# qiskit-community/adapt-aqc

Measured on AMD Instinct MI355X. Metric: overlap+gradient evals/sec, 50-qubit MPS chi=64, 1/2/4/8 MI355X, higher is better.
Workload: dtype c128

## Files before the change

### adaptaqc_amd/_lib.py

```python
import atexit
import ctypes
import os
import threading

import numpy as np

_HERE = os.path.dirname(os.path.abspath(__file__))
LIB_PATH = os.environ.get("AQC_LIB") or os.path.join(_HERE, "libaqchip.so")

OP_DTYPE = np.dtype(
    [("nq", "<i4"), ("q0", "<i4"), ("q1", "<i4"), ("flags", "<i4"), ("m", "<f8", (32,))], align=True
)
assert OP_DTYPE.itemsize == 272
OP_KRAUS1 = 1
OP_MEASURE1 = 2
OP_KRAUS2 = 3

EXPORTS = (
    "aqc_last_error", "aqc_version", "aqc_init", "aqc_finalize", "aqc_timing_enable",
    "aqc_timing_query", "aqc_timing_reset",
    "aqc_sv_create", "aqc_sv_destroy", "aqc_sv_reset", "aqc_sv_copy", "aqc_sv_apply", "aqc_sv_plan",
    "aqc_sv_amp0", "aqc_sv_z_all", "aqc_sv_get", "aqc_sv_set",
    "aqc_mps_create", "aqc_mps_destroy", "aqc_mps_set_truncation", "aqc_mps_set_vidal",
    "aqc_mps_get_vidal", "aqc_mps_get_dims", "aqc_mps_copy", "aqc_mps_copy_batch", "aqc_mps_apply",
    "aqc_mps_apply_batch", "aqc_mps_apply_sort_batch", "aqc_mps_apply_sort_batch_async", "aqc_mps_apply_batch_async", "aqc_mps_check_batch", "aqc_mps_sort", "aqc_mps_sort_batch", "aqc_mps_overlap_zero",
    "aqc_mps_overlap_zero_batch", "aqc_mps_dot", "aqc_mps_z_all", "aqc_mps_amps_hw1", "aqc_mps_z_all_batch", "aqc_mps_z_sum_batch", "aqc_mps_zero_hw1_batch",
    "aqc_mps_amps_hw1_batch",
    "aqc_pair_grads", "aqc_pair_grads_batch", "aqc_argmax_scaled", "aqc_argmax_scaled_batch", "aqc_mps_jacobi_stats",
    "aqc_mps_set_jacobi_tol", "aqc_mps_set_jacobi_stop", "aqc_mps_set_fused_chain", "aqc_mps_chain_ticks", "aqc_svd_debug",
    "aqc_sv_pair_rdms", "aqc_mps_pair_rdms", "aqc_mps_pair_rdms_batch", "aqc_entanglement_measures",
    "aqc_sv_transition", "aqc_mps_product_fit", "aqc_mps_set_svd_path", "aqc_svd_gram_ticks", "aqc_bj_ticks",
    "aqc_sweep_set_chain_mode", "aqc_stream_join", "aqc_stream_wait", "aqc_svd_gram_stats", "aqc_env_ticks",
    "aqc_comm_unique_id", "aqc_comm_init", "aqc_comm_destroy", "aqc_comm_rank", "aqc_allgather_f64",
    "aqc_allgather_f64_host", "aqc_allreduce_max_f64", "aqc_svd_gram_big_stats", "aqc_svd_gram_big_ticks",
    "aqc_gb_set_spin_limit", "aqc_gb_set_tail", "aqc_gb_set_stages", "aqc_debug_hog", "aqc_pool_stats",
    "aqc_scratch_stats", "aqc_mps_set_chain_epilogue", "aqc_mps_chain_epilogue_stats",
    "aqc_env_fallbacks", "aqc_env_set_single", "aqc_env_set_spin_limit",
    "aqc_sv_sample", "aqc_mps_sample", "aqc_sample_uniforms", "aqc_sv_traj_sample",
    "aqc_sv_traj_pair_tomo", "aqc_sv_traj_pauli_counts", "aqc_mps_traj_sample", "aqc_mps_traj_plan", "aqc_mps_traj_set_batch",
    "aqc_mps_traj_pair_tomo", "aqc_mps_traj_tomo_plan", "aqc_mps_traj_set_readout_batch",
    "aqc_sv_pauli_expect", "aqc_mps_pauli_expect", "aqc_mps_pauli_expect_batch",
    "aqc_pair_tomo_probs", "aqc_concurrence_bound_probs", "aqc_multinomial_counts", "aqc_tomo_fit",
)


class AqcError(RuntimeError):
    pass


_lock = threading.Lock()
_lib = None
_initialised_device = None

_P = ctypes.c_void_p
_I = ctypes.c_int
_D = ctypes.c_double
_DP = ctypes.POINTER(ctypes.c_double)
_IP = ctypes.POINTER(ctypes.c_int)

_SIGS = {
    "aqc_last_error": ([], ctypes.c_char_p),
    "aqc_version": ([], _I),
    "aqc_init": ([_I], _I),
    "aqc_finalize": ([], _I),
    "aqc_timing_enable": ([_I], _I),
    "aqc_timing_query": ([ctypes.c_char_p, _DP, ctypes.POINTER(ctypes.c_int64), _DP, _DP], _I),
    "aqc_timing_reset": ([], _I),
    "aqc_sv_create": ([_I, ctypes.POINTER(_P)], _I),
    "aqc_sv_destroy": ([_P], _I),
    "aqc_sv_reset": ([_P], _I),
    "aqc_sv_copy": ([_P, _P], _I),
    "aqc_sv_apply": ([_P, _P, _I], _I),
    "aqc_sv_plan": ([_I, _P, _I, _P], _I),
    "aqc_sv_amp0": ([_P, _DP, _DP], _I),
    "aqc_sv_z_all": ([_P, _DP], _I),
    "aqc_sv_get": ([_P, _P], _I),
    "aqc_sv_set": ([_P, _P], _I),
    "aqc_mps_create": ([_I, _I, _D, _I, ctypes.POINTER(_P)], _I),
    "aqc_mps_destroy": ([_P], _I),
    "aqc_mps_set_truncation": ([_P, _D, _I], _I),
    "aqc_mps_set_vidal": ([_P, _P, _P, _P], _I),
    "aqc_mps_get_vidal": ([_P, _P, _P, _P], _I),
    "aqc_mps_get_dims": ([_P, _P], _I),
    "aqc_mps_copy": ([_P, _P], _I),
    "aqc_mps_copy_batch": ([_P, _P, _I], _I),
    "aqc_mps_apply": ([_P, _P, _I], _I),
    "aqc_mps_apply_batch": ([_P, _I, _P, _P], _I),
    "aqc_mps_apply_sort_batch": ([_P, _I, _P, _P], _I),
    "aqc_mps_apply_sort_batch_async": ([_P, _I, _P, _P], _I),
    "aqc_mps_apply_batch_async": ([_P, _I, _P, _P], _I),
    "aqc_mps_check_batch": ([_P, _I], _I),
    "aqc_mps_sort": ([_P], _I),
    "aqc_mps_sort_batch": ([_P, _I], _I),
    "aqc_mps_overlap_zero": ([_P, _DP, _DP], _I),
    "aqc_mps_overlap_zero_batch": ([_P, _I, _P], _I),
    "aqc_mps_dot": ([_P, _P, _DP, _DP], _I),
    "aqc_mps_z_all": ([_P, _P], _I),
    "aqc_mps_amps_hw1": ([_P, _P], _I),
    "aqc_mps_z_all_batch": ([_P, _I, _P], _I),
    "aqc_mps_z_sum_batch": ([_P, _P, _I, _P], _I),
    "aqc_mps_zero_hw1_batch": ([_P, _P, _I, _P, _P], _I),
    "aqc_mps_amps_hw1_batch": ([_P, _I, _P], _I),
    "aqc_pair_grads": ([_P, _P, _P, _I, _P, _P, _P, _I, _P, _I], _I),
    "aqc_pair_grads_batch": ([_P, _I, _P, _P, _I, _P, _P, _P, _I, _P, _I], _I),
    "aqc_argmax_scaled": ([_P, _P, _I, _I, _IP], _I),
    "aqc_argmax_scaled_batch": ([_P, _I, _P, _I, _I, _P], _I),
    "aqc_mps_jacobi_stats": ([_P, _IP], _I),
    "aqc_mps_set_jacobi_tol": ([_D], _I),
    "aqc_mps_set_jacobi_stop": ([_D], _I),
    "aqc_mps_set_fused_chain": ([_I], _I),
    "aqc_mps_chain_ticks": ([_P], _I),
    "aqc_mps_set_chain_epilogue": ([_I], _I),
    "aqc_mps_chain_epilogue_stats": ([_P], _I),
    "aqc_svd_debug": ([_P, _I, _I, _I, _I, _P, _P, _P, _P], _I),
    "aqc_sv_pair_rdms": ([_P, _P, _I, _P], _I),
    "aqc_mps_pair_rdms": ([_P, _P, _I, _P], _I),
    "aqc_mps_pair_rdms_batch": ([_P, _I, _P, _I, _P, _I], _I),
    "aqc_entanglement_measures": ([_P, _I, _I, _P, _I], _I),
    "aqc_sv_transition": ([_P, _P, _I, _P], _I),
    "aqc_mps_product_fit": ([_P, _P, _I, _I, _I, _D, _DP, _IP], _I),
    "aqc_mps_set_svd_path": ([_I, _I], _I),
    "aqc_svd_gram_ticks": ([_P], _I),
    "aqc_bj_ticks": ([_P], _I),
    "aqc_sweep_set_chain_mode": ([_I], _I),
    "aqc_stream_join": ([_P], _I),
    "aqc_stream_wait": ([_P], _I),
    "aqc_svd_gram_stats": ([_P], _I),
    "aqc_env_ticks": ([_P], _I),
    "aqc_comm_unique_id": ([ctypes.c_char_p], _I),
    "aqc_comm_init": ([ctypes.c_char_p, _I, _I, ctypes.POINTER(_P)], _I),
    "aqc_comm_destroy": ([_P], _I),
    "aqc_comm_rank": ([_P, _IP, _IP], _I),
    "aqc_allgather_f64": ([_P, _P, _P, ctypes.c_size_t], _I),
    "aqc_allgather_f64_host": ([_P, _P, _P, ctypes.c_size_t], _I),
    "aqc_allreduce_max_f64": ([_P, _DP], _I),
    "aqc_svd_gram_big_stats": ([_P], _I),
    "aqc_svd_gram_big_ticks": ([_P], _I),
    "aqc_gb_set_spin_limit": ([_D], _I),
    "aqc_env_fallbacks": ([ctypes.POINTER(ctypes.c_longlong)], _I),
    "aqc_env_set_single": ([_I], _I),
    "aqc_env_set_spin_limit": ([_D], _I),
    "aqc_gb_set_tail": ([_I], _I),
    "aqc_gb_set_stages": ([_I], _I),
    "aqc_debug_hog": ([_I, _D], _I),
    "aqc_pool_stats": ([_P], _I),
    "aqc_scratch_stats": ([_P], _I),
    "aqc_sv_sample": ([_P, _I, ctypes.c_uint64, ctypes.c_uint64, _P, _P], _I),
    "aqc_mps_sample": ([_P, _I, ctypes.c_uint64, ctypes.c_uint64, _P, _P], _I),
    "aqc_sample_uniforms": ([ctypes.c_uint64, ctypes.c_uint64, _I, _I, _P], _I),
    "aqc_sv_traj_sample": ([_I, _P, _I, _I, ctypes.c_uint64, ctypes.c_uint64, _P, _P, _P], _I),
    "aqc_sv_traj_pair_tomo": ([_I, _P, _I, _P, _I, _P, _I, ctypes.c_uint64, ctypes.c_uint64, _P, _P, _P], _I),
    "aqc_sv_traj_pauli_counts": ([_I, _P, _I, _P, _I, _P, _I, ctypes.c_uint64, ctypes.c_uint64, _P, _P, _P, _P], _I),
    "aqc_mps_traj_sample": ([_I, _I, _D, _I, _P, _I, _I, ctypes.c_uint64, ctypes.c_uint64, _P, _P, _P], _I),
    "aqc_mps_traj_plan": ([_I, _P, _I, _P, _P, _I], _I),
    "aqc_mps_traj_set_batch": ([_I], _I),
    "aqc_mps_traj_pair_tomo": ([_I, _I, _D, _I, _P, _I, _P, _I, _P, _I, ctypes.c_uint64, ctypes.c_uint64, _P, _P, _P], _I),
    "aqc_mps_traj_tomo_plan": ([_I, _P, _I, _P, _P, _I], _I),
    "aqc_mps_traj_set_readout_batch": ([_I], _I),
    "aqc_sv_pauli_expect": ([_P, _P, _P, _I, _P], _I),
    "aqc_mps_pauli_expect": ([_P, _P, _I, _P], _I),
    "aqc_mps_pauli_expect_batch": ([_P, _I, _P, _I, _P], _I),
    "aqc_pair_tomo_probs": ([_P, _I, _P, _I], _I),
    "aqc_concurrence_bound_probs": ([_P, _I, _P, _I], _I),
    "aqc_multinomial_counts": ([_P, _I, _I, _I, ctypes.c_uint64, ctypes.c_uint64, _P, _P], _I),
    "aqc_tomo_fit": ([_P, _I, _P, _I], _I),
# ... 121 lines not shown
```

### adaptaqc_amd/csrc/mps.hip

```cpp
#include <algorithm>
#include <cmath>
#include <chrono>
#include <cstring>
#include <atomic>
#include <cstdlib>
#include <mutex>
#include <thread>
#include <unordered_set>

#include "aqc_gemm.h"
#include "mps_internal.h"

using aqc::cplx;

namespace aqc {

namespace {
std::mutex g_mps_stream_mu;
hipStream_t g_mps_streams[64] = {nullptr};
void release_mps_streams() {
  std::lock_guard<std::mutex> lk(g_mps_stream_mu);
  for (auto& s : g_mps_streams)
    if (s) (void)hipStreamDestroy(s), s = nullptr;
}
}

hipStream_t mps_stream() {
  int dev = 0;
  hipGetDevice(&dev);
  std::lock_guard<std::mutex> lk(g_mps_stream_mu);
  if (!g_mps_streams[dev]) {
    hipStreamCreateWithFlags(&g_mps_streams[dev], hipStreamNonBlocking);
    note_device(dev);
    on_finalize(release_mps_streams);
  }
  return g_mps_streams[dev];
}

hipStream_t mps_stream_if_any(int dev) {
  if (dev < 0 || dev >= 64) return nullptr;
  std::lock_guard<std::mutex> lk(g_mps_stream_mu);
  return g_mps_streams[dev];
}

StagingRing& staging_ring() {
  static PerDevice<StagingRing> rings;
  return rings.here();
}

}

namespace {

using aqc::fresh_tid;
using aqc::StagingLease;
using aqc::wave_sum_d;

constexpr int kT = 256;
constexpr double kChop = 1e-16;
constexpr int kMaxSweeps = 60;
double g_jacobi_tol_factor = 1.0;
constexpr double kDefaultTinyT = 1e-6;
constexpr double kStopCos = 3e-13;
constexpr int kStopCosSweeps = 30;
double g_jacobi_tiny_t = kDefaultTinyT;
constexpr double kJacobiNoise = 0.0;
bool g_fused_chain = true;
int g_chain_epilogue = [] {
  const char* e = std::getenv("AQC_CHAIN_EPILOGUE");
  const int v = e ? std::atoi(e) : 1;
  return v >= 0 && v <= 2 ? v : 1;
}();
int g_chain_min_states = 32;
constexpr int kChainLdsBytes = 4 * (int)sizeof(aqc::GemmLds);

struct OneSiteJob {
  cplx* g;
  const int* dims;
  int cap;
  int pad;
  cplx u[4];
};

using aqc::TwoSiteJob;
using aqc::kMaxCap;
using aqc::kSigMax;
using aqc::kSigTail;
using aqc::kSigLen;

__global__ void k_mps_zero(cplx* gam, double* lam, int* dims, int n, int cap) {
  const size_t ss = (size_t)2 * cap * cap;
  for (int i = blockIdx.x * blockDim.x + threadIdx.x; i < n; i += gridDim.x * blockDim.x) {
    gam[(size_t)i * ss] = aqc::cmk(1.0, 0.0);
  }
  for (int b = blockIdx.x * blockDim.x + threadIdx.x; b <= n; b += gridDim.x * blockDim.x) {
    lam[(size_t)b * cap] = 1.0;
    dims[b] = 1;
  }
}

__global__ __launch_bounds__(kT) void k_1q(const OneSiteJob* __restrict__ jobs) {
  const OneSiteJob& j = jobs[blockIdx.y];
  const int cl = j.dims[0], cr = j.dims[1];
  const int cap = j.cap;
  const size_t half = (size_t)cap * cap;
  for (int e = blockIdx.x * kT + threadIdx.x; e < cl * cr; e += gridDim.x * kT) {
    const int l = e / cr, r = e % cr;
    const size_t o = (size_t)l * cap + r;
    const cplx a0 = aqc::ldg(j.g + o), a1 = aqc::ldg(j.g + half + o);
    aqc::stg(j.g + o, aqc::cfma(j.u[1], a1, aqc::cmul(j.u[0], a0)));
    aqc::stg(j.g + half + o, aqc::cfma(j.u[3], a1, aqc::cmul(j.u[2], a0)));
  }
}

__global__ __launch_bounds__(kT) void k_theta(const TwoSiteJob* __restrict__ jobs, int nj) {
  int jb, tile;
  if (!aqc::xcd_job_block(nj, jb, tile)) return;
  const TwoSiteJob& j = jobs[jb];
  const int chl = j.dims[0], chm = j.dims[1], chr = j.dims[2];
  const int cap = j.cap;
  const int tiles_r = (cap + 15) / 16;
  const int l0 = (tile / tiles_r) * 16, r0 = (tile % tiles_r) * 16;
  if (l0 >= chl || r0 >= chr) return;
  __shared__ cplx As[2][16][17];
// ... 951 lines not shown
  aqc::d4_t cr[2][2], ci[2][2];
  if (!tr) {
    aqc::block_cgemm_tile<true, true, false>(
        mb, nb, kh, 0, 0,
        [&](int kk, int R) {
          return klo + R < L ? aqc::cconj(aqc::ldg(W + (size_t)perm[r0 + kk] * L + klo + R)) : aqc::cmk(0, 0);
        },
        [&](int R, int c) { return klo + R < L ? aqc::ldg(th + (size_t)(c0 + c) * M + klo + R) : aqc::cmk(0, 0); }, lds, lt,
        active, cr, ci);
  } else {
    aqc::block_cgemm_tile<false, true, false>(
        mb, nb, kh, 0, 0,
        [&](int R, int c) { return klo + c < L ? aqc::ldg(th + (size_t)(klo + c) * M + r0 + R) : aqc::cmk(0, 0); },
        [&](int c, int kk) { return klo + c < L ? aqc::ldg(W + (size_t)perm[c0 + kk] * L + klo + c) : aqc::cmk(0, 0); }, lds,
        lt, active, cr, ci);
  }
  cplx* part = xbuf + blk * (64 * 64);
  const int wave = lt >> 6, lane = lt & 63;
  const int wr = (wave >> 1) * 32, wc = (wave & 1) * 32, li = lane & 15, lk = lane >> 4;
  if (active && h == 1) {
#pragma unroll
    for (int r = 0; r < 2; ++r)
#pragma unroll
      for (int c = 0; c < 2; ++c)
#pragma unroll
        for (int q = 0; q < 4; ++q)
          part[(wr + 16 * r + lk + 4 * q) * 64 + wc + 16 * c + li] = aqc::cmk(cr[r][c][q], ci[r][c][q]);
  }
  __syncthreads();
  if (active && h == 0) {
#pragma unroll
    for (int r = 0; r < 2; ++r)
#pragma unroll
      for (int c = 0; c < 2; ++c)
#pragma unroll
        for (int q = 0; q < 4; ++q) {
          const int i = wr + 16 * r + lk + 4 * q, jj = wc + 16 * c + li;
          if (i < mb && jj < nb) {
            const cplx o = part[i * 64 + jj];
            const cplx v = aqc::cmk(cr[r][c][q] + o.x, ci[r][c][q] + o.y);
            if (!tr) {
              const int kq = r0 + i, cc = c0 + jj, s2 = cc / chr, rr = cc % chr;
              const double sk = aqc::ldg(ss + kq), d = sk * sk * aqc::ldg(j.lr + rr);
              aqc::stg(j.gq + s2 * half + (size_t)kq * cap + rr, d != 0.0 ? aqc::cscale(v, 1.0 / d) : aqc::cmk(0, 0));
            } else {
              const int Rr = r0 + i, kq = c0 + jj, s1 = Rr / chl, l = Rr % chl;
              const double sk = aqc::ldg(ss + kq), d = sk * sk * aqc::ldg(j.ll + l);
              aqc::stg(j.gp + s1 * half + (size_t)l * cap + kq, d != 0.0 ? aqc::cscale(v, 1.0 / d) : aqc::cmk(0, 0));
            }
          }
        }
  }
}
__device__ __forceinline__ void chain_split(const TwoSiteJob& j, bool copied) {
  const int tid = fresh_tid();
  if (!copied) split_copy_body(j, tid, 1024);
  split_gemm_chain(j, tid);
}

__global__ __launch_bounds__(1024) void k_chain(const ChainJob* __restrict__ chains, const TwoSiteJob* __restrict__ two,
                                                const OneSiteJob* __restrict__ one, int epi) {
  const ChainJob& c = chains[blockIdx.x];
  const int tid = fresh_tid();
  __shared__ unsigned long long tk[6];
  if (tid == 0) tk[0] = tk[1] = tk[2] = tk[3] = tk[4] = tk[5] = 0;
  auto tick = [&](int ph) {
    if (tid == 0) {
      const unsigned long long t = __builtin_amdgcn_s_memtime();
      if (ph >= 0) tk[ph] += t - tk[5];
      tk[5] = t;
    }
  };
  tick(-1);
  for (int o = 0; o < c.nops; ++o) {
    const int code = __builtin_amdgcn_readfirstlane(c.ops[o]);
    if (code < 0) {
      one_site_body(one[-code - 1], tid, 1024);
      __syncthreads();
      tick(4);
      continue;
    }
    const TwoSiteJob& j = two[code];
#if AQC_THETA_MFMA
    chain_theta_mfma(j);
#else
    chain_theta(j);
#endif
    __syncthreads();
    tick(0);
    const int done = __builtin_amdgcn_readfirstlane(chain_jacobi(j, epi));
    __syncthreads();
    tick(1);
    if (done == 0) chain_rank(j);
    __syncthreads();
    tick(2);
    chain_split(j, done == 2);
    __syncthreads();
    tick(3);
  }
  if (tid == 0)
    for (int ph = 0; ph < 5; ++ph) atomicAdd(&g_chain_ticks[ph], tk[ph]);
}

using aqc::DevOp;
using aqc::Scheduler;
using aqc::KrausJob;
using aqc::TrajCtx;
using aqc::run_waves;

template <class F>
void parallel_states(int ns, F&& f) {
  static const int kThreads = [] {
    const char* e = std::getenv("AQC_HOST_THREADS");
    const int v = e ? std::atoi(e) : 1;
    return v < 1 ? 1 : (v > 64 ? 64 : v);
  }();
  const int nt = std::min(kThreads, ns / 32);
  if (nt <= 1) {
    for (int s = 0; s < ns; ++s) f(s);
    return;
  }
  std::vector<std::thread> th;
  th.reserve(nt - 1);
  for (int t = 1; t < nt; ++t)
    th.emplace_back([&f, t, nt, ns] {
      for (int s = t; s < ns; s += nt) f(s);
    });
  for (int s = 0; s < ns; s += nt) f(s);
  for (auto& x : th) x.join();
}

bool distinct_handles(aqc_mps_t* hs, int ns) {
  std::unordered_set<const void*> seen;
  seen.reserve(2 * ns);
  for (int s = 0; s < ns; ++s)
    if (!seen.insert(hs[s]).second) return false;
  return true;
}

int validate_ops(aqc_mps_t h, const aqc_op_t* ops, int nops) {
  for (int i = 0; i < nops; ++i) {
    const aqc_op_t& o = ops[i];
    AQC_REQUIRE(o.nq == 1 || o.nq == 2, "aqc_mps_apply: only 1- and 2-qubit ops are supported");
    AQC_REQUIRE(o.q0 >= 0 && o.q0 < h->d.n, "aqc_mps_apply: qubit index out of range");
    if (o.nq == 2) AQC_REQUIRE(o.q1 >= 0 && o.q1 < h->d.n && o.q1 != o.q0, "aqc_mps_apply: bad second qubit");
  }
  return AQC_OK;
}

// ... 603 lines not shown

int aqc_mps_set_jacobi_tol(double factor) {
  AQC_REQUIRE(factor > 0, "aqc_mps_set_jacobi_tol: factor must be positive");
  g_jacobi_tol_factor = factor;
  return AQC_OK;
}

int aqc_svd_gram_ticks(double* out) {
  AQC_REQUIRE(out, "aqc_svd_gram_ticks: null argument");
  unsigned long long t[12];
  AQC_HIP_CHECK(hipMemcpyFromSymbol(t, HIP_SYMBOL(g_gram_ticks), sizeof(t)));
  for (int i = 0; i < 12; ++i) out[i] = (double)t[i];
  unsigned long long z[12] = {0, 0, 0, 0, 0, 0, 0, 0, 0, 0, 0, 0};
  AQC_HIP_CHECK(hipMemcpyToSymbol(HIP_SYMBOL(g_gram_ticks), z, sizeof(z)));
  return AQC_OK;
}

int aqc_svd_gram_stats(double* out) {
  AQC_REQUIRE(out, "aqc_svd_gram_stats: null argument");
  unsigned long long t[6];
  AQC_HIP_CHECK(hipMemcpyFromSymbol(t, HIP_SYMBOL(g_gram_stats), sizeof(t)));
  for (int i = 0; i < 6; ++i) out[i] = (double)t[i];
  unsigned long long z[6] = {0, 0, 0, 0, 0, 0};
  AQC_HIP_CHECK(hipMemcpyToSymbol(HIP_SYMBOL(g_gram_stats), z, sizeof(z)));
  return AQC_OK;
}

int aqc_mps_set_svd_path(int gram, int debug_max_chi) {
  AQC_REQUIRE(gram >= 0 && gram <= 1, "aqc_mps_set_svd_path: gram must be 0 or 1");
  g_svd_gram = gram;
  g_debug_max_chi = debug_max_chi;
  return AQC_OK;
}


int aqc_mps_set_jacobi_stop(double tiny_t) {
  AQC_REQUIRE(tiny_t < 1e-3, "aqc_mps_set_jacobi_stop: tiny_t must be < 1e-3 (<= 0 restores the default)");
  g_jacobi_tiny_t = tiny_t > 0 ? tiny_t : kDefaultTinyT;
  return AQC_OK;
}

int aqc_mps_chain_ticks(double* out) {
  AQC_REQUIRE(out, "aqc_mps_chain_ticks: null argument");
  unsigned long long t[5] = {0, 0, 0, 0, 0};
  AQC_HIP_CHECK(hipStreamSynchronize(aqc::mps_stream()));
  AQC_HIP_CHECK(hipMemcpyFromSymbol(t, HIP_SYMBOL(g_chain_ticks), sizeof(t)));
  const unsigned long long z[5] = {0, 0, 0, 0, 0};
  AQC_HIP_CHECK(hipMemcpyToSymbol(HIP_SYMBOL(g_chain_ticks), z, sizeof(z)));
  for (int i = 0; i < 5; ++i) out[i] = (double)t[i];
  return AQC_OK;
}

int aqc_mps_set_chain_epilogue(int mode) {
  AQC_REQUIRE(mode >= 0 && mode <= 2, "aqc_mps_set_chain_epilogue: 0, 1 or 2");
  g_chain_epilogue = mode;
  return AQC_OK;
}

int aqc_mps_chain_epilogue_stats(double* out) {
  AQC_REQUIRE(out, "aqc_mps_chain_epilogue_stats: null argument");
  unsigned long long t[2] = {0, 0};
  AQC_HIP_CHECK(hipStreamSynchronize(aqc::mps_stream()));
  AQC_HIP_CHECK(hipMemcpyFromSymbol(t, HIP_SYMBOL(g_epi_stats), sizeof(t)));
  const unsigned long long z[2] = {0, 0};
  AQC_HIP_CHECK(hipMemcpyToSymbol(HIP_SYMBOL(g_epi_stats), z, sizeof(z)));
  for (int i = 0; i < 2; ++i) out[i] = (double)t[i];
  return AQC_OK;
}

int aqc_mps_set_fused_chain(int on) {
  AQC_REQUIRE(on >= 0 && on <= 2, "aqc_mps_set_fused_chain: 0, 1 or 2");
  g_fused_chain = on != 0;
  g_chain_min_states = on == 2 ? 1 : 32;
  return AQC_OK;
}


int aqc_mps_set_truncation(aqc_mps_t h, double threshold, int max_chi) {
  AQC_REQUIRE(h, "aqc_mps_set_truncation: null handle");
  h->thr = threshold;
  h->max_chi = max_chi;
  return AQC_OK;
}

int aqc_mps_set_vidal(aqc_mps_t h, const int* dims, const double* gammas, const double* lambdas) {
  AQC_REQUIRE(h && dims && gammas && lambdas, "aqc_mps_set_vidal: null argument");
  const int n = h->d.n, cap = h->d.cap;
  AQC_REQUIRE(dims[0] == 1 && dims[n] == 1, "aqc_mps_set_vidal: dims[0] and dims[n] must be 1");
  for (int b = 0; b <= n; ++b) {
    if (dims[b] < 1 || dims[b] > cap) {
      aqc::set_error("aqc_mps_set_vidal: bond dimension exceeds chi_cap");
      return AQC_ERR_ARG;
    }
  }
  std::vector<cplx> g((size_t)n * 2 * cap * cap, aqc::cmk(0, 0));
  std::vector<double> l((size_t)(n + 1) * cap, 0.0);
  size_t off = 0;
  for (int i = 0; i < n; ++i)
    for (int s = 0; s < 2; ++s)
      for (int a = 0; a < dims[i]; ++a)
        for (int b = 0; b < dims[i + 1]; ++b, ++off)
          g[(size_t)i * 2 * cap * cap + (size_t)s * cap * cap + (size_t)a * cap + b] =
              aqc::cmk(gammas[2 * off], gammas[2 * off + 1]);
  l[0] = 1.0;
  l[(size_t)n * cap] = 1.0;
  size_t lo = 0;
  for (int b = 1; b < n; ++b)
    for (int k = 0; k < dims[b]; ++k) l[(size_t)b * cap + k] = lambdas[lo++];
  hipStream_t st = aqc::mps_stream();
  AQC_HIP_CHECK(hipStreamSynchronize(st));
// ... 245 lines not shown
```

### adaptaqc_amd/csrc/svd_gram.h

```cpp
#pragma once

constexpr int kGramMaxK = 128;
constexpr int kGramNarrowK = 64;
constexpr double kGramRelFloor = 1e-9;
__device__ unsigned long long g_gram_ticks[12];
static_assert(kGramNarrowK == 64, "S5: the narrow inverse iteration (tid < K) stays on wave 0");
__device__ unsigned long long g_gram_stats[6];
__device__ unsigned long long g_epi_stats[2];

__device__ __forceinline__ int rank_rule(const TwoSiteJob& j, const double* sv, int n, double tail, double& norm) {
  int k = 0;
  for (int i = 0; i < n; ++i)
    if (sv[i] * sv[i] > kChop) ++k;
  if (k < 1) k = 1;
  if (j.max_chi > 0 && k > j.max_chi) k = j.max_chi;
  while (k > 1 && tail + sv[k - 1] * sv[k - 1] < j.thr) {
    tail += sv[k - 1] * sv[k - 1];
    --k;
  }
  if (k > j.cap) {
    k = j.cap;
    atomicOr(&j.flags[0], 1);
  }
  double nn = 0.0;
// ... 186 lines not shown
        for (int row = lane; row < C; row += 64) zb[row * ZS + i] = fma(-dp, zb[row * ZS + jj], zb[row * ZS + i]);
      }
      const double n2 = normalise(i);
      if (n2 > 0.5 || again == 2) break;
      asm volatile("s_waitcnt lgkmcnt(0)" ::: "memory");
      __builtin_amdgcn_wave_barrier();
      if (lane == 0) {
        double yp = 0.0;
        for (int row = 0; row < C; ++row) {
          const int rm = max(row - 1, 0);
          yp = fma(-s_e[rm] * ldd(rm, i), yp, zb[row * ZS + i]);
          zb[row * ZS + i] = yp;
        }
        double zn = 0.0;
        for (int row = C - 1; row >= 0; --row) {
          const double d = ldd(row, i);
          zn = fma(-s_e[min(row, C - 2)] * d, zn, zb[row * ZS + i] * d);
          zb[row * ZS + i] = zn;
        }
      }
      asm volatile("s_waitcnt lgkmcnt(0)" ::: "memory");
      __builtin_amdgcn_wave_barrier();
      normalise(i);
    }
  }
}

template <int ZS>
__device__ __forceinline__ double rayleigh(int i, int C, const double* zb, const double* s_d, const double* s_e) {
  double s2a = 0.0, s2b = 0.0;
  int r0 = 0;
  constexpr int U = 8;
  for (; r0 + U <= C; r0 += U) {
    double zz[U + 1], dd[U], ee[U];
#pragma unroll
    for (int u = 0; u <= U; ++u) zz[u] = zb[min(r0 + u, C - 1) * ZS + i];
#pragma unroll
    for (int u = 0; u < U; ++u) dd[u] = s_d[r0 + u], ee[u] = r0 + u < C - 1 ? s_e[r0 + u] : 0.0;
#pragma unroll
    for (int u = 0; u < U; ++u) {
      s2a = fma(dd[u] * zz[u], zz[u], s2a);
      s2b = fma(2.0 * ee[u] * zz[u], zz[u + 1], s2b);
    }
  }
  for (; r0 < C; ++r0) {
    const double z = zb[r0 * ZS + i];
    s2a = fma(s_d[r0] * z, z, s2a);
    if (r0 < C - 1) s2b = fma(2.0 * s_e[r0] * z, zb[(r0 + 1) * ZS + i], s2b);
  }
  const double s2 = s2a + s2b;
  return s2 > 0.0 ? s2 : 0.0;
}

__device__ __forceinline__ void s6_back(const TwoSiteJob& j, cplx* hh, int C, int K, int c0, aqc::d4_t (&vre)[2],
                                        aqc::d4_t (&vim)[2], const double* s_sig2, int tid, int lane, int wave,
                                        int wave_s, bool copy = false, bool gtr = false, const int* s_fk = nullptr) {
  extern __shared__ double2 xbuf[];
  const int nt = wave & 3, mg = wave >> 2, li = lane & 15, lk = lane >> 4;
  cplx* Yl = xbuf;
  cplx* Pw = Yl + 2048;
  cplx* Tl = Pw + 12 * 256;
  cplx* W2l = Tl + 3 * 256 + 16 * 64;
  auto fetch_y = [&](int k0, int nb, cplx (&y)[2]) {
#pragma unroll
    for (int u = 0; u < 2; ++u) {
      const int e = tid + 1024 * u, row = e >> 4, i = e & 15, k = k0 + i;
      y[u] = (i < nb && row > k && row < C) ? aqc::ldg(hh + (size_t)k * (2 * C - k - 1) / 2 + (row - k - 1))
                                            : aqc::cmk(0, 0);
    }
  };
  cplx ynx[2];
  {
    const int k1 = C - 1, k0 = k1 > 16 ? k1 - 16 : 0;
    fetch_y(k0, k1 - k0, ynx);
  }
  __syncthreads();
  for (int k1 = C - 1; k1 > 0; k1 -= 16) {
    const int k0 = k1 > 16 ? k1 - 16 : 0;
#pragma unroll
    for (int u = 0; u < 2; ++u) {
      const int e = tid + 1024 * u, row = e >> 4, i = e & 15;
      Yl[row * 16 + (i ^ (row & 15))] = ynx[u];
    }
    if (tid < 256) {
      const gdbl_t* tp = (const gdbl_t*)(const double*)(hh + kTfacOff + (size_t)((C - 1 - k1) >> 4) * 512 + 256 + tid);
      Tl[(tid >> 4) * 17 + (tid & 15)] = aqc::cmk(__hip_atomic_load(tp, __ATOMIC_RELAXED, __HIP_MEMORY_SCOPE_AGENT),
                                                  __hip_atomic_load(tp + 1, __ATOMIC_RELAXED, __HIP_MEMORY_SCOPE_AGENT));
    }
    __syncthreads();
    aqc::d4_t wr, wi;
    {
      aqc::d4_t p1 = {0, 0, 0, 0}, p2 = {0, 0, 0, 0}, p3 = {0, 0, 0, 0};
#pragma unroll
      for (int t = 0; t < 2; ++t) {
        if (32 * mg + 16 * t + 15 > k0) {
#pragma unroll
          for (int s = 0; s < 4; ++s) {
            const int row = 32 * mg + 16 * t + 4 * s + lk;
            const cplx y = Yl[row * 16 + (li ^ (row & 15))];
            p1 = __builtin_amdgcn_mfma_f64_16x16x4f64(y.x, vre[t][s], p1, 0, 0, 0);
            p2 = __builtin_amdgcn_mfma_f64_16x16x4f64(-y.y, vim[t][s], p2, 0, 0, 0);
            p3 = __builtin_amdgcn_mfma_f64_16x16x4f64(y.x - y.y, vre[t][s] + vim[t][s], p3, 0, 0, 0);
          }
        }
      }
#pragma unroll
      for (int q = 0; q < 4; ++q) wr[q] = p1[q] - p2[q], wi[q] = p3[q] - p1[q] - p2[q];
    }
    if (mg > 0) {
#pragma unroll
      for (int q = 0; q < 4; ++q) Pw[((mg - 1) * 4 + nt) * 256 + (lk + 4 * q) * 16 + li] = aqc::cmk(wr[q], wi[q]);
    }
    __syncthreads();
    if (mg == 0) {
      aqc::d4_t br, bi, p1 = {0, 0, 0, 0}, p2 = {0, 0, 0, 0}, p3 = {0, 0, 0, 0};
#pragma unroll
      for (int q = 0; q < 4; ++q) {
        const int b = lk + 4 * q;
        cplx w = aqc::cmk(wr[q], wi[q]);
#pragma unroll
        for (int m = 0; m < 3; ++m) w = aqc::cadd(w, Pw[(m * 4 + nt) * 256 + b * 16 + li]);
        br[q] = w.x;
        bi[q] = w.y;
      }
#pragma unroll
      for (int q = 0; q < 4; ++q) {
        const cplx t = Tl[li * 17 + 4 * q + lk];
        p1 = __builtin_amdgcn_mfma_f64_16x16x4f64(t.x, br[q], p1, 0, 0, 0);
        p2 = __builtin_amdgcn_mfma_f64_16x16x4f64(t.y, bi[q], p2, 0, 0, 0);
        p3 = __builtin_amdgcn_mfma_f64_16x16x4f64(t.x + t.y, br[q] + bi[q], p3, 0, 0, 0);
      }
#pragma unroll
      for (int q = 0; q < 4; ++q) W2l[(lk + 4 * q) * 64 + 16 * nt + li] = aqc::cmk(p1[q] - p2[q], p3[q] - p1[q] - p2[q]);
    }
    __syncthreads();
    if (k0 > 0) {
      const int n1 = k0, n0 = n1 > 16 ? n1 - 16 : 0;
      fetch_y(n0, n1 - n0, ynx);
    }
    const int vl_ = fresh_lane();
    const int vmg = wave_s >> 2, vnt = wave_s & 3, vli = vl_ & 15, vlk = vl_ >> 4;
#pragma unroll
    for (int t = 0; t < 2; ++t) {
      if (32 * vmg + 16 * t + 15 > k0) {
        const int row = 32 * vmg + 16 * t + vli;
        aqc::d4_t p1 = {0, 0, 0, 0}, p2 = {0, 0, 0, 0};
#pragma unroll
        for (int s = 0; s < 4; ++s) {
          const int b = 4 * s + vlk;
          const cplx y = Yl[row * 16 + (b ^ (row & 15))];
          const cplx w = W2l[b * 64 + 16 * vnt + vli];
          p1 = __builtin_amdgcn_mfma_f64_16x16x4f64(y.x, w.x, p1, 0, 0, 0);
          p2 = __builtin_amdgcn_mfma_f64_16x16x4f64(y.y, w.y, p2, 0, 0, 0);
          vim[t] = __builtin_amdgcn_mfma_f64_16x16x4f64(-(y.x + y.y), w.x + w.y, vim[t], 0, 0, 0);
        }
#pragma unroll
        for (int q = 0; q < 4; ++q) vre[t][q] += p2[q] - p1[q], vim[t][q] += p1[q] + p2[q];
      }
    }
    __syncthreads();
  }
  {
    const int col = c0 + 16 * nt + li;
    if (col < K) {
      const double sg = sqrt(s_sig2[col]);
#pragma unroll
      for (int t = 0; t < 2; ++t) {
#pragma unroll
        for (int q = 0; q < 4; ++q) {
          const int row = 32 * mg + 16 * t + lk + 4 * q;
          if (row < C) aqc::stg(j.work + (size_t)col * C + row, aqc::cmk(vre[t][q] * sg, vim[t][q] * sg));
        }
      }
    }
    if (copy && col < *s_fk) {
      const int chs = C >> 1;
      const size_t half = (size_t)j.cap * j.cap;
      const double sg = sqrt(s_sig2[col]);
      const double* lo = gtr ? j.ll : j.lr;
#pragma unroll
      for (int t = 0; t < 2; ++t) {
#pragma unroll
        for (int q = 0; q < 4; ++q) {
          const int row = 32 * mg + 16 * t + lk + 4 * q;
          if (row < C) {
            const int s = row >= chs, o = row - s * chs;
            const double d = sg * aqc::ldg(lo + o);
            cplx w = aqc::cmk(vre[t][q] * sg, vim[t][q] * sg);
            if (!gtr) w = aqc::cconj(w);
            w = d != 0.0 ? aqc::cscale(w, 1.0 / d) : aqc::cmk(0, 0);
            if (gtr) aqc::stg(j.gp + s * half + (size_t)o * j.cap + col, w);
            else aqc::stg(j.gq + s * half + (size_t)col * j.cap + o, w);
          }
        }
      }
    }
  }
}

__device__ __noinline__ void s5_wide(int i, int C, const double* s_d, const double* s_e, const double* s_e2,
                                     double lam, double tn, double* zb, double* Db) {
  for (int row = 0; row < C; ++row) {
    unsigned int h = (unsigned int)(row * 2654435761u) ^ (unsigned int)((i + 1) * 40503u);
    h ^= h >> 13;
    h *= 0x5bd1e995u;
    h ^= h >> 15;
    zb[row * 128 + i] = (double)(h & 0xFFFFFu) * (2.0 / 1048576.0) - 1.0;
  }
  auto ldd = [&](int row) {
    return __hip_atomic_load((const gdbl_t*)(Db + row * 128 + i), __ATOMIC_RELAXED, __HIP_MEMORY_SCOPE_AGENT);
  };
  constexpr int U = 8;
  const double itn = 1.0 / fmax(tn, 1e-300), lamn = lam * itn;
// ... 785 lines not shown
        zn = fma(-e * d, zn, y * d);
        zb[row * 64 + i] = zn;
        n2 = fma(zn, zn, n2);
      };
      int r1 = C - 1;
      for (; r1 - U + 1 >= 0; r1 -= U) {
        double yy[U], ee[U], dd[U];
#pragma unroll
        for (int u = 0; u < U; ++u) {
          const int row = r1 - u;
          yy[u] = zb[row * 64 + i], ee[u] = s_e[min(row, C - 2)], dd[u] = Db[row * 64 + i];
        }
#pragma unroll
        for (int u = 0; u < U; ++u) bwd_row(r1 - u, yy[u], ee[u], dd[u]);
      }
      for (; r1 >= 0; --r1) bwd_row(r1, zb[r1 * 64 + i], s_e[min(r1, C - 2)], Db[r1 * 64 + i]);
      const double rs = __builtin_amdgcn_rsq(n2);
      sc = rs * fma(-0.5 * n2 * rs, rs, 1.5);
    }
    {
      int r0 = 0;
      for (; r0 + U <= C; r0 += U) {
        double zz[U];
#pragma unroll
        for (int u = 0; u < U; ++u) zz[u] = zb[(r0 + u) * 64 + i];
#pragma unroll
        for (int u = 0; u < U; ++u) zb[(r0 + u) * 64 + i] = zz[u] * sc;
      }
      for (; r0 < C; ++r0) zb[r0 * 64 + i] *= sc;
    }
    if (tid == 0) atomicAdd(&g_gram_ticks[7], __builtin_amdgcn_s_memtime() - t_last);
  }
  else if ((wave & 3) != 0 && wave - 1 - (wave >> 2) < ((C - 1 + 15) >> 4)) {
    s6_factors(wave - 1 - (wave >> 2), C, hh, s_tau, lane);
  }
  __syncthreads();
  if (wave == 0)
    gs_clusters<64>(K, C, zb, s_lam, s_e, s_tn, lane, [&](int row, int i) { return Db[row * 64 + i]; });
  __syncthreads();
  if (tid < K) s_sig2[tid] = rayleigh<64>(tid, C, zb, s_d, s_e);
  __syncthreads();
  tick(3);
  const int nt = wave & 3, mg = wave >> 2, li = lane & 15, lk = lane >> 4;
  aqc::d4_t vre[2], vim[2];
#pragma unroll
  for (int t = 0; t < 2; ++t) {
#pragma unroll
    for (int q = 0; q < 4; ++q) {
      const int row = 32 * mg + 16 * t + lk + 4 * q, col = 16 * nt + li;
      vre[t][q] = (row < C && col < K) ? zb[row * 64 + col] : 0.0;
      vim[t][q] = 0.0;
    }
  }
  if (epi == 2 && j.qr == 0) epi = 1;
  if (epi && !s_cert && wave == 0) {
    const double sg = lane < K ? sqrt(s_sig2[lane]) : 0.0;
    s_err[lane] = sg;
    const bool ok = __ballot(lane >= K - 1 || sg >= __shfl_down(sg, 1)) == ~0ull;
    __builtin_amdgcn_wave_barrier();
    double nrm = 0.0;
    int k = 0;
    if (lane == 0) {
      if (ok) {
        k = rank_rule(j, s_err, K, s_tail, nrm);
        *(__attribute__((address_space(1))) int*)(j.dims + 1) = k;
      }
      s_fk = k;
      atomicAdd(&g_epi_stats[ok ? 0 : 1], 1ull);
    }
    k = __builtin_amdgcn_readfirstlane(k);
    nrm = uniform_d(nrm);
    if (lane < k) {
      aqc::stg(j.lm + lane, sg / nrm);
      *(__attribute__((address_space(1))) int*)(j.perm + lane) = lane;
      aqc::stg(j.sig + lane + kSigMax, sg);
    }
  }
  s6_back(j, hh, C, K, 0, vre, vim, s_sig2, tid, lane, wave, wave_s, epi == 2 && !s_cert, tr, &s_fk);
  tick(4);
  }
  const int fk = (epi && !s_cert && K <= kGramNarrowK) ? __builtin_amdgcn_readfirstlane(s_fk) : 0;
  for (int c = tid; c < C; c += 1024) aqc::stg(j.sig + c, c < K ? sqrt(s_sig2[c]) : 0.0);
  if (tid == 0) aqc::stg(j.sig + kSigTail, fk ? 0.0 : s_tail);
  tick(5);
  if (s_cert) return 2;
  if (tid == 0) {
    atomicMax(&j.flags[2], 1);
    atomicAdd(&g_gram_stats[1], 1ull);
  }
  return fk ? 2 + epi : 1;
}

__device__ __noinline__ bool gram_certified(const TwoSiteJob& j) {
  const int tid = fresh_tid();
  __shared__ double s_s2[128];
  __shared__ int s_k;
  const int M = 2 * j.dims[0], N = 2 * j.dims[2], C = M < N ? M : N;
  if (tid == 0) s_k = 0;
  __syncthreads();
  if (tid < C) {
    const double sg = aqc::ldg(j.sig + tid);
    s_s2[tid] = sg * sg;
    if (sg > 0.0) atomicMax(&s_k, tid + 1);
  }
  __syncthreads();
  if (tid == 0) atomicAdd(&g_gram_stats[4], 1ull);
  const double cs = gram_cert128(j, C, s_k, s_s2);
  const bool ok = cs < 0.5 * aqc::kReduceChop;
  if (tid == 0) {
    atomicAdd(&g_gram_stats[ok ? 5 : 3], 1ull);
    if (ok) {
      atomicMax(&j.flags[2], 1);
      atomicAdd(&g_gram_stats[1], 1ull);
    } else {
      aqc::stg(j.sig + kSigTail, 0.0);
    }
  }
  __syncthreads();
  return ok;
}

__global__ __launch_bounds__(1024) void k_svd_gram(const TwoSiteJob* __restrict__ jobs) {
  const TwoSiteJob& j = jobs[blockIdx.x];
  const int g = j.gram ? gram_svd_body(j, 0) : 0;
  if (g == 1) return;
  __syncthreads();
  if (g == 2 && gram_certified(j)) return;
  jacobi_reg_body<128, 8, 16>(j);
}
```

### include/aqc_hip_diag.h

```cpp
#ifndef AQC_HIP_DIAG_H
#define AQC_HIP_DIAG_H

#include "aqc_hip.h"

#ifdef __cplusplus
extern "C" {
#endif

int aqc_mps_jacobi_stats(aqc_mps_t h, int* max_sweeps);
int aqc_mps_set_jacobi_tol(double factor);
int aqc_mps_set_jacobi_stop(double tiny_t);
int aqc_mps_set_svd_path(int gram, int debug_max_chi);
int aqc_svd_gram_ticks(double* out);
int aqc_svd_gram_stats(double* out);
int aqc_env_ticks(double* out);
int aqc_env_fallbacks(long long* out);
int aqc_env_set_single(int on);
int aqc_env_set_spin_limit(double us);
int aqc_bj_ticks(double* out);
int aqc_svd_gram_big_stats(double* out);
int aqc_svd_gram_big_ticks(double* out);
int aqc_gb_set_spin_limit(double us);
int aqc_gb_set_tail(int on);
int aqc_gb_set_stages(int n);
int aqc_debug_hog(int nblocks, double ms);
int aqc_pool_stats(double* out);
int aqc_scratch_stats(double* out);
int aqc_mps_set_fused_chain(int on);
int aqc_mps_set_chain_epilogue(int mode);
int aqc_mps_chain_epilogue_stats(double* out);
int aqc_mps_chain_ticks(double* out);
int aqc_svd_debug(const double* theta, int m, int n, int variant, int stop_after_qr, double* w_out,
                  double* sig_out, int* perm_out, int* sweeps);
int aqc_sweep_set_chain_mode(int mode);
int aqc_sample_uniforms(uint64_t seed, uint64_t run, int nshots, int nper, double* out);
#ifdef __cplusplus
}
#endif
#endif
```

Baseline: 8.186 million.

## Keep SVD right vectors in LDS and fuse the split GEMM into chain epilogue

Adds a new chain epilogue mode 3 and makes it the default. In this mode the Gram-SVD back-transform leaves the V factor and precomputed reciprocal scales (sigma, left and right lambdas) in shared memory instead of writing them to global memory. The chain split step then reads V from LDS, writes one factor directly, and computes the other with an in-kernel f64 MFMA 3-multiply complex GEMM against theta. This removes a global round trip and the separate split copy and GEMM passes. In exchange it uses more LDS and adds code paths that depend on capacity assumptions (V up to 128x64).

```diff
diff --git a/adaptaqc_amd/_lib.py b/adaptaqc_amd/_lib.py
--- a/adaptaqc_amd/_lib.py
+++ b/adaptaqc_amd/_lib.py
@@ -34,7 +34,7 @@
     "aqc_comm_unique_id", "aqc_comm_init", "aqc_comm_destroy", "aqc_comm_rank", "aqc_allgather_f64",
     "aqc_allgather_f64_host", "aqc_allreduce_max_f64", "aqc_svd_gram_big_stats", "aqc_svd_gram_big_ticks",
     "aqc_gb_set_spin_limit", "aqc_gb_set_tail", "aqc_gb_set_stages", "aqc_debug_hog", "aqc_pool_stats",
-    "aqc_scratch_stats", "aqc_mps_set_chain_epilogue", "aqc_mps_chain_epilogue_stats",
+    "aqc_scratch_stats", "aqc_mps_set_chain_epilogue", "aqc_mps_get_chain_epilogue", "aqc_mps_chain_epilogue_stats",
     "aqc_env_fallbacks", "aqc_env_set_single", "aqc_env_set_spin_limit",
     "aqc_sv_sample", "aqc_mps_sample", "aqc_sample_uniforms", "aqc_sv_traj_sample",
     "aqc_sv_traj_pair_tomo", "aqc_sv_traj_pauli_counts", "aqc_mps_traj_sample", "aqc_mps_traj_plan", "aqc_mps_traj_set_batch",
@@ -111,6 +111,7 @@
     "aqc_mps_set_fused_chain": ([_I], _I),
     "aqc_mps_chain_ticks": ([_P], _I),
     "aqc_mps_set_chain_epilogue": ([_I], _I),
+    "aqc_mps_get_chain_epilogue": ([], _I),
     "aqc_mps_chain_epilogue_stats": ([_P], _I),
     "aqc_svd_debug": ([_P, _I, _I, _I, _I, _P, _P, _P, _P], _I),
     "aqc_sv_pair_rdms": ([_P, _P, _I, _P], _I),
diff --git a/adaptaqc_amd/csrc/mps.hip b/adaptaqc_amd/csrc/mps.hip
--- a/adaptaqc_amd/csrc/mps.hip
+++ b/adaptaqc_amd/csrc/mps.hip
@@ -68,8 +68,8 @@
 bool g_fused_chain = true;
 int g_chain_epilogue = [] {
   const char* e = std::getenv("AQC_CHAIN_EPILOGUE");
-  const int v = e ? std::atoi(e) : 1;
-  return v >= 0 && v <= 2 ? v : 1;
+  const int v = e ? std::atoi(e) : 3;
+  return v >= 0 && v <= 3 ? v : 3;
 }();
 int g_chain_min_states = 32;
 constexpr int kChainLdsBytes = 4 * (int)sizeof(aqc::GemmLds);
@@ -1127,9 +1127,103 @@
         }
   }
 }
-__device__ __forceinline__ void chain_split(const TwoSiteJob& j, bool copied) {
+template <bool TR>
+__device__ __forceinline__ void split_lds_body(const TwoSiteJob& j, int tid) {
+  extern __shared__ double2 xbuf[];
+  const cplx* Vl = xbuf;
+  const double* rcp = reinterpret_cast<const double*>(xbuf + kVlElems);
+  const int chl = j.dims[0], k = j.dims[1], chr = j.dims[2];
+  const int M = 2 * chl, N = 2 * chr;
+  const int C = TR ? N : M;
+  const int cap = j.cap;
+  const size_t half = (size_t)cap * cap;
+  if (TR) {
+    for (int e = tid; e < N * k; e += 1024) {
+      const int cc = e % N, kk = e / N;
+      const int s2 = cc >= chr, r = cc - s2 * chr;
+      const double f = rcp[kVlRcpSig + kk] != 0.0 ? rcp[kVlRcpLr + r] : 0.0;
+      const cplx v = Vl[kVlPos(cc, kk)];
+      aqc::stg(j.gq + s2 * half + (size_t)kk * cap + r, aqc::cmk(v.x * f, -v.y * f));
+    }
+  } else {
+    for (int e = tid; e < M * k; e += 1024) {
+      const int kk = e % k, R = e / k;
+      const int s1 = R >= chl, l = R - s1 * chl;
+      const double f = rcp[kVlRcpSig + kk] != 0.0 ? rcp[kVlRcpLl + l] : 0.0;
+      const cplx v = Vl[kVlPos(R, kk)];
+      aqc::stg(j.gp + s1 * half + (size_t)l * cap + kk, aqc::cmk(v.x * f, v.y * f));
+    }
+  }
+  const int wave = __builtin_amdgcn_readfirstlane(tid >> 6), lane = tid & 63;
+  const int li = lane & 15, lk = lane >> 4;
+  const int rt = wave >> 1, ct = 2 * (wave & 1);
+  const int outer = TR ? M : N;
+  if (16 * rt >= outer) return;
+  const int m = 16 * rt + li;
+  const bool mok = m < outer;
+  const cplx* tp = j.theta + (TR ? (size_t)lk * M + m : (size_t)m * M + lk);
+  const size_t ts = TR ? (size_t)4 * M : 4;
+  auto ldt = [&](int s) { return (mok && 4 * s + lk < C) ? aqc::ldg(tp + s * ts) : aqc::cmk(0, 0); };
+  aqc::d4_t p1[2], p2[2], p3[2];
+#pragma unroll
+  for (int u = 0; u < 2; ++u) p1[u] = p2[u] = p3[u] = aqc::d4_t{0, 0, 0, 0};
+  auto kstep = [&](int s, cplx t) {
+    const int row = 4 * s + lk;
+    const double tsum = t.x + t.y;
+#pragma unroll
+    for (int u = 0; u < 2; ++u) {
+      const cplx v = Vl[kVlPos(row, 16 * (ct + u) + li)];
+      if (TR) {
+        p1[u] = __builtin_amdgcn_mfma_f64_16x16x4f64(t.x, v.x, p1[u], 0, 0, 0);
+        p2[u] = __builtin_amdgcn_mfma_f64_16x16x4f64(t.y, v.y, p2[u], 0, 0, 0);
+        p3[u] = __builtin_amdgcn_mfma_f64_16x16x4f64(tsum, v.x + v.y, p3[u], 0, 0, 0);
+      } else {
+        p1[u] = __builtin_amdgcn_mfma_f64_16x16x4f64(v.x, t.x, p1[u], 0, 0, 0);
+        p2[u] = __builtin_amdgcn_mfma_f64_16x16x4f64(v.y, t.y, p2[u], 0, 0, 0);
+        p3[u] = __builtin_amdgcn_mfma_f64_16x16x4f64(v.x - v.y, tsum, p3[u], 0, 0, 0);
+      }
+    }
+  };
+  const int nks = (C + 3) >> 2;
+  cplx t0 = ldt(0), t1 = ldt(1);
+  for (int s = 0; s < nks; s += 2) {
+    const cplx n0 = ldt(s + 2), n1 = ldt(s + 3);
+    kstep(s, t0);
+    if (s + 1 < nks) kstep(s + 1, t1);
+    t0 = n0;
+    t1 = n1;
+  }
+#pragma unroll
+  for (int u = 0; u < 2; ++u) {
+#pragma unroll
+    for (int q = 0; q < 4; ++q) {
+      const double re = TR ? p1[u][q] - p2[u][q] : p1[u][q] + p2[u][q];
+      const double im = TR ? p3[u][q] - p1[u][q] - p2[u][q] : p3[u][q] - p1[u][q] + p2[u][q];
+      const int kq = 16 * (ct + u) + (TR ? li : lk + 4 * q);
+      const int o = 16 * rt + (TR ? lk + 4 * q : li);
+      if (kq < k && o < outer) {
+        const int ch = TR ? chl : chr;
+        const int s = o >= ch, b = o - s * ch;
+        const double f1 = rcp[kVlRcpSig + kq], f2 = rcp[(TR ? kVlRcpLl : kVlRcpLr) + b];
+        const cplx g = aqc::cmk(re * f1 * f2, im * f1 * f2);
+        if (TR) aqc::stg(j.gp + s * half + (size_t)b * cap + kq, g);
+        else aqc::stg(j.gq + s * half + (size_t)kq * cap + b, g);
+      }
+    }
+  }
+}
+__device__ __forceinline__ void split_lds_chain(const TwoSiteJob& j, int tid) {
+  const bool tr = 2 * j.dims[0] >= 2 * j.dims[2];
+  if (tr) split_lds_body<true>(j, tid);
+  else split_lds_body<false>(j, tid);
+}
+__device__ __forceinline__ void chain_split(const TwoSiteJob& j, int done) {
   const int tid = fresh_tid();
-  if (!copied) split_copy_body(j, tid, 1024);
+  if (done == 3) {
+    split_lds_chain(j, tid);
+    return;
+  }
+  if (done != 2) split_copy_body(j, tid, 1024);
   split_gemm_chain(j, tid);
 }
 
@@ -1169,7 +1263,7 @@
     if (done == 0) chain_rank(j);
     __syncthreads();
     tick(2);
-    chain_split(j, done == 2);
+    chain_split(j, done);
     __syncthreads();
     tick(3);
   }
@@ -1879,10 +1973,12 @@
 }
 
 int aqc_mps_set_chain_epilogue(int mode) {
-  AQC_REQUIRE(mode >= 0 && mode <= 2, "aqc_mps_set_chain_epilogue: 0, 1 or 2");
+  AQC_REQUIRE(mode >= 0 && mode <= 3, "aqc_mps_set_chain_epilogue: 0, 1, 2 or 3");
   g_chain_epilogue = mode;
   return AQC_OK;
 }
+
+int aqc_mps_get_chain_epilogue(void) { return g_chain_epilogue; }
 
 int aqc_mps_chain_epilogue_stats(double* out) {
   AQC_REQUIRE(out, "aqc_mps_chain_epilogue_stats: null argument");
diff --git a/adaptaqc_amd/csrc/svd_gram.h b/adaptaqc_amd/csrc/svd_gram.h
--- a/adaptaqc_amd/csrc/svd_gram.h
+++ b/adaptaqc_amd/csrc/svd_gram.h
@@ -262,9 +262,37 @@
   return s2 > 0.0 ? s2 : 0.0;
 }
 
+constexpr int kVlElems = 128 * 64;
+constexpr int kVlRcpSig = 0, kVlRcpLl = 64, kVlRcpLr = 128, kVlRcpLen = 192;
+static_assert(kChainLdsBytes >= kVlElems * 16 + kVlRcpLen * 8, "V and the reciprocals exceed the chain's LDS");
+__device__ __forceinline__ int kVlPos(int row, int col) { return row * 64 + (col ^ (row & 15)); }
+
+__device__ __noinline__ void s6_leave_lds(const TwoSiteJob& j, aqc::d4_t vre0, aqc::d4_t vre1, aqc::d4_t vim0,
+                                          aqc::d4_t vim1, int K, const double* s_sig2) {
+  extern __shared__ double2 xbuf[];
+  cplx* Vl = xbuf;
+  double* rcp = reinterpret_cast<double*>(xbuf + kVlElems);
+  const int tid = fresh_tid(), lane = tid & 63, wave = tid >> 6;
+  const int nt = wave & 3, mg = wave >> 2, li = lane & 15, lk = lane >> 4;
+#pragma unroll
+  for (int q = 0; q < 4; ++q) {
+    Vl[kVlPos(32 * mg + lk + 4 * q, 16 * nt + li)] = aqc::cmk(vre0[q], vim0[q]);
+    Vl[kVlPos(32 * mg + 16 + lk + 4 * q, 16 * nt + li)] = aqc::cmk(vre1[q], vim1[q]);
+  }
+  if (tid < kVlRcpLen) {
+    const int o = tid & 63;
+    double x;
+    if (tid < kVlRcpLl) x = o < K ? sqrt(s_sig2[o]) : 0.0;
+    else if (tid < kVlRcpLr) x = o < j.dims[0] ? aqc::ldg(j.ll + o) : 0.0;
+    else x = o < j.dims[2] ? aqc::ldg(j.lr + o) : 0.0;
+    rcp[tid] = x != 0.0 ? 1.0 / x : 0.0;
+  }
+}
+
 __device__ __forceinline__ void s6_back(const TwoSiteJob& j, cplx* hh, int C, int K, int c0, aqc::d4_t (&vre)[2],
                                         aqc::d4_t (&vim)[2], const double* s_sig2, int tid, int lane, int wave,
-                                        int wave_s, bool copy = false, bool gtr = false, const int* s_fk = nullptr) {
+                                        int wave_s, bool copy = false, bool gtr = false, const int* s_fk = nullptr,
+                                        bool lds = false) {
   extern __shared__ double2 xbuf[];
   const int nt = wave & 3, mg = wave >> 2, li = lane & 15, lk = lane >> 4;
   cplx* Yl = xbuf;
@@ -369,6 +397,10 @@
       }
     }
     __syncthreads();
+  }
+  if (lds && *s_fk > 0) {
+    s6_leave_lds(j, vre[0], vre[1], vim[0], vim[1], K, s_sig2);
+    return;
   }
   {
     const int col = c0 + 16 * nt + li;
@@ -1260,7 +1292,7 @@
       vim[t][q] = 0.0;
     }
   }
-  if (epi == 2 && j.qr == 0) epi = 1;
+  if (epi >= 2 && j.qr == 0) epi = 1;
   if (epi && !s_cert && wave == 0) {
     const double sg = lane < K ? sqrt(s_sig2[lane]) : 0.0;
     s_err[lane] = sg;
@@ -1284,7 +1316,8 @@
       aqc::stg(j.sig + lane + kSigMax, sg);
     }
   }
-  s6_back(j, hh, C, K, 0, vre, vim, s_sig2, tid, lane, wave, wave_s, epi == 2 && !s_cert, tr, &s_fk);
+  s6_back(j, hh, C, K, 0, vre, vim, s_sig2, tid, lane, wave, wave_s, epi == 2 && !s_cert, tr, &s_fk,
+          epi == 3 && !s_cert);
   tick(4);
   }
   const int fk = (epi && !s_cert && K <= kGramNarrowK) ? __builtin_amdgcn_readfirstlane(s_fk) : 0;
diff --git a/include/aqc_hip_diag.h b/include/aqc_hip_diag.h
--- a/include/aqc_hip_diag.h
+++ b/include/aqc_hip_diag.h
@@ -28,6 +28,7 @@
 int aqc_scratch_stats(double* out);
 int aqc_mps_set_fused_chain(int on);
 int aqc_mps_set_chain_epilogue(int mode);
+int aqc_mps_get_chain_epilogue(void);
 int aqc_mps_chain_epilogue_stats(double* out);
 int aqc_mps_chain_ticks(double* out);
 int aqc_svd_debug(const double* theta, int m, int n, int variant, int stop_after_qr, double* w_out,
```

New measurement: 8.640 million (median of 6 runs). 1.06x the previous value.
